# zhangxinsong-nlp/XFM

Measured on AMD Instinct MI355X. Metric: image-text pairs/sec fwd+bwd, XFM-base 224px/30tok, higher is better.
Workload: dtype bf16; 1 GPU; Pretrain.py full multimodal step (ITC+ITM+MLM+MIM), XFM-base, synthetic 224px images + 30-token captions, random init; units_per_gpu=64, global_batch=64, dropout=True, ordered_reductions=True, grad_allreduce=False, parallelism=dp1, image_res=224

## Files before the change

### xfm_amd/csrc/gemm_tn_256.hip

```cpp
__device__ __forceinline__ void wait_younger(int y) {
  if (y >= 3) asm volatile("s_waitcnt vmcnt(6)" ::: "memory");
  else if (y == 2) asm volatile("s_waitcnt vmcnt(4)" ::: "memory");
  else if (y == 1) asm volatile("s_waitcnt vmcnt(2)" ::: "memory");
  else asm volatile("s_waitcnt vmcnt(0)" ::: "memory");
}

struct Tn256Seg {
  const bf16* dY; const bf16* X;
  unsigned ldy, ldx;
  int n0, k0, mbeg, nk;
  bool do_bias;
  int rows;
};
__device__ __attribute__((aligned(16))) const unsigned tn_zero16[4] = {0u, 0u, 0u, 0u};

template <bool RAGGED>
__device__ __forceinline__ void tn256_mainloop(const Tn256Seg& sg, char* smem, f32x4 (&acc)[8][4], f32x4 (&bacc)[2]) {
  constexpr int UNIT = 64 * 256, BUF = 4 * UNIT;
  const int tid = threadIdx.x, lane = tid & 63, w = tid >> 6;
  const int wr = w >> 2, wc = w & 3;
  const int lr = lane & 15, lg = lane >> 4;
  const int n0 = sg.n0, k0 = sg.k0, mbeg = sg.mbeg, nk = sg.nk;
  const int total = 4 * nk;
  const bool do_bias = sg.do_bias;

  unsigned soff[4][2];
  int doff[4][2];
#pragma unroll
  for (int i = 0; i < 2; ++i) {
    const int b = i * 8 + w;
    const int r = 4 * b + (lane >> 4);
    const int c = ((lane & 15) ^ swz_t(r)) * 8;
    const unsigned rowy = (unsigned)(mbeg + r) * (unsigned)sg.ldy, rowx = (unsigned)(mbeg + r) * (unsigned)sg.ldx;
    soff[0][i] = rowy + n0 + (c >> 6) * 128 + (c & 63);
    soff[3][i] = rowy + n0 + (c >> 6) * 128 + 64 + (c & 63);
    soff[1][i] = rowx + k0 + (c >> 5) * 64 + (c & 31);
    soff[2][i] = rowx + k0 + (c >> 5) * 64 + 32 + (c & 31);
    doff[0][i] = 0 * UNIT + b * 1024;
    doff[1][i] = 1 * UNIT + b * 1024;
    doff[2][i] = 2 * UNIT + b * 1024;
    doff[3][i] = 3 * UNIT + b * 1024;
  }
  auto issue = [&](int s) {
    if (s >= total) return;
    const int kt = s >> 2, j = s & 3;
    char* base = smem + (kt & 1) * BUF;
    const bool isy = (j == 0 || j == 3);
    const bf16* src = (isy ? sg.dY : sg.X) + (size_t)kt * 64 * (size_t)(isy ? sg.ldy : sg.ldx);
#pragma unroll
    for (int i = 0; i < 2; ++i) {
      const unsigned so = j == 0 ? soff[0][i] : j == 1 ? soff[1][i] : j == 2 ? soff[2][i] : soff[3][i];
      const int dofs = j == 0 ? doff[0][i] : j == 1 ? doff[1][i] : j == 2 ? doff[2][i] : doff[3][i];
      const unsigned lds_addr = (unsigned)(uintptr_t)LDS_PTR(void, base) + (unsigned)__builtin_amdgcn_readfirstlane(dofs);
      const bf16* ptr = src + (size_t)so;
      if (RAGGED && kt * 64 + 4 * (i * 8 + w) + (lane >> 4) >= sg.rows) ptr = reinterpret_cast<const bf16*>(tn_zero16);
      asm volatile("s_mov_b32 m0, %1\n\ts_nop 0\n\tglobal_load_lds_dwordx4 %0, off" ::"v"(ptr), "s"(lds_addr) : "memory", "m0");
    }
  };

#pragma unroll
  for (int i = 0; i < 8; ++i)
#pragma unroll
    for (int j = 0; j < 4; ++j) acc[i][j] = f32x4{0.f, 0.f, 0.f, 0.f};
  bacc[0] = bacc[1] = f32x4{0.f, 0.f, 0.f, 0.f};
  bf16x8 ones;
#pragma unroll
  for (int i = 0; i < 8; ++i) ones[i] = f2bf(1.0f);

  const int lrow = 8 * lg + (lr >> 2);
  const int tsw = swz_t(lrow);
  int offa[4], offb[2];
#pragma unroll
  for (int f = 0; f < 4; ++f) {
    const int col = wr * 64 + f * 16 + 4 * (lr & 3);
    offa[f] = lrow * 256 + (((col >> 3) ^ tsw) << 4) + (col & 7) * 2;
  }
#pragma unroll
  for (int f = 0; f < 2; ++f) {
    const int col = wc * 32 + f * 16 + 4 * (lr & 3);
    offb[f] = lrow * 256 + (((col >> 3) ^ tsw) << 4) + (col & 7) * 2;
  }
  auto tr_pair = [&](const char* p) {
    const s16x4 lo = __builtin_amdgcn_ds_read_tr16_b64_v4i16(LDS_PTR(s16x4, p));
    const s16x4 hi = __builtin_amdgcn_ds_read_tr16_b64_v4i16(LDS_PTR(s16x4, p + 1024));
    union { struct { s16x4 a, b; } s; bf16x8 v; } u;
    u.s.a = lo;
    u.s.b = hi;
    return u.v;
  };
  bf16x8 xa[4][2], wb0[2][2], wb1[2][2];
  auto read_a = [&](const char* unit) {
#pragma unroll
    for (int f = 0; f < 4; ++f) {
      xa[f][0] = tr_pair(unit + offa[f]);
      xa[f][1] = tr_pair(unit + offa[f] + 8192);
    }
  };
  auto read_b = [&](const char* unit, bf16x8 (&wb)[2][2]) {
#pragma unroll
    for (int f = 0; f < 2; ++f) {
      wb[f][0] = tr_pair(unit + offb[f]);
      wb[f][1] = tr_pair(unit + offb[f] + 8192);
    }
  };
#define XFM_TQUAD(MH, NH, WB)                                                                                    \
  do {                                                                                                           \
    __builtin_amdgcn_s_setprio(1);                                                                               \
    _Pragma("unroll") for (int ks = 0; ks < 2; ++ks)                                                             \
    _Pragma("unroll") for (int m = 0; m < 4; ++m)                                                                \
    _Pragma("unroll") for (int n = 0; n < 2; ++n)                                                                \
      acc[MH * 4 + m][NH * 2 + n] =                                                                              \
          __builtin_amdgcn_mfma_f32_16x16x32_bf16(xa[m][ks], WB[n][ks], acc[MH * 4 + m][NH * 2 + n], 0, 0, 0);  \
    __builtin_amdgcn_s_setprio(0);                                                                               \
  } while (0)
#define XFM_TBIAS(H)                                                                                             \
  do {                                                                                                           \
    if (do_bias) {                                                                                               \
      _Pragma("unroll") for (int f = 0; f < 4; ++f)                                                              \
        if (f == wc) {                                                                                           \
          bacc[H] = __builtin_amdgcn_mfma_f32_16x16x32_bf16(xa[f][0], ones, bacc[H], 0, 0, 0);                  \
          bacc[H] = __builtin_amdgcn_mfma_f32_16x16x32_bf16(xa[f][1], ones, bacc[H], 0, 0, 0);                  \
        }                                                                                                        \
    }                                                                                                            \
  } while (0)

#pragma unroll
  for (int s = 0; s < 5; ++s) issue(s);
  wait_younger((total - 1 < 4 ? total - 1 : 4) - 1);
  XFM_BAR();
  if (wr == 1) XFM_BAR();

  for (int kt = 0; kt < nk; ++kt) {
    const char* buf = smem + (kt & 1) * BUF;
    const int ph = 4 * kt;
    int last;
    issue(ph + 5);
    read_a(buf + 0 * UNIT);
    read_b(buf + 1 * UNIT, wb0);
    last = ph + 5 < total ? ph + 5 : total - 1;
    wait_younger(last - (ph + 2));
    XFM_BAR();
    XFM_TQUAD(0, 0, wb0);
    XFM_TBIAS(0);
    XFM_BAR();
    issue(ph + 6);
    read_b(buf + 2 * UNIT, wb1);
    last = ph + 6 < total ? ph + 6 : total - 1;
    wait_younger(last - (ph + 3));
    XFM_BAR();
    XFM_TQUAD(0, 1, wb1);
    XFM_BAR();
    issue(ph + 7);
    read_a(buf + 3 * UNIT);
    XFM_BAR();
    XFM_TQUAD(1, 1, wb1);
    XFM_TBIAS(1);
    XFM_BAR();
    issue(ph + 8);
    last = ph + 8 < total ? ph + 8 : total - 1;
    wait_younger(last - (ph + 5) < 0 ? 0 : last - (ph + 5));
    XFM_BAR();
    XFM_TQUAD(1, 0, wb0);
    XFM_BAR();
  }
  if (wr == 0) XFM_BAR();
#undef XFM_TQUAD
#undef XFM_TBIAS

}

template <bool ATOMIC>
__device__ __forceinline__ void tn256_bias_out(float* dbias, int n0, const f32x4 (&bacc)[2]) {
  const int lane = threadIdx.x & 63, w = threadIdx.x >> 6, wr = w >> 2, wc = w & 3, lr = lane & 15, lg = lane >> 4;
  if (lr != 0) return;
#pragma unroll
  for (int h = 0; h < 2; ++h)
#pragma unroll
    for (int i = 0; i < 4; ++i) {
      float* d = dbias + n0 + wr * 128 + h * 64 + wc * 16 + 4 * lg + i;
      if (ATOMIC) atomicAdd(d, bacc[h][i]);
      else *d += bacc[h][i];
    }
}
__device__ __forceinline__ void tn256_bias_part(float* part, const f32x4 (&bacc)[2]) {
  const int lane = threadIdx.x & 63, w = threadIdx.x >> 6, wr = w >> 2, wc = w & 3, lr = lane & 15, lg = lane >> 4;
  if (lr != 0) return;
#pragma unroll
  for (int h = 0; h < 2; ++h) *reinterpret_cast<f32x4*>(part + wr * 128 + h * 64 + wc * 16 + 4 * lg) = bacc[h];
}
__device__ __forceinline__ void tn256_store_partial(float* ws, long slot, const f32x4 (&acc)[8][4]) {
  const int lane = threadIdx.x & 63, w = threadIdx.x >> 6;
  f32x4* wsp = reinterpret_cast<f32x4*>(ws) + ((slot * 8 + w) * 32) * 64 + lane;
#pragma unroll
  for (int nt = 0; nt < 8; ++nt)
#pragma unroll
    for (int kt = 0; kt < 4; ++kt) wsp[(nt * 4 + kt) * 64] = acc[nt][kt];
}
template <bool ATOMIC>
__device__ __forceinline__ void tn256_add_out(float* dW, long ldw, int n0, int k0, const f32x4 (&acc)[8][4]) {
  const int lane = threadIdx.x & 63, w = threadIdx.x >> 6, wr = w >> 2, wc = w & 3, lr = lane & 15, lg = lane >> 4;
#pragma unroll
  for (int nt = 0; nt < 8; ++nt)
#pragma unroll
    for (int kt = 0; kt < 4; ++kt) {
      const int k = k0 + wc * 64 + kt * 16 + lr;
#pragma unroll
      for (int rgi = 0; rgi < 4; ++rgi) {
        const int n = n0 + wr * 128 + nt * 16 + 4 * lg + rgi;
        if (ATOMIC) atomicAdd(dW + (long)n * ldw + k, acc[nt][kt][rgi]);
        else dW[(long)n * ldw + k] += acc[nt][kt][rgi];
      }
    }
}

__global__ __launch_bounds__(512) void gemm_tn_256_kernel(GemmTN g) {
  extern __shared__ __attribute__((aligned(16))) char smem[];
  const int tiles_k = g.K / 256, tiles_n = g.N / 256;
  const int per_split = tiles_k * tiles_n;
  const int wg = xcd_remap(blockIdx.x, gridDim.x);
  const int split = wg / per_split, t = wg % per_split;
  const int n0 = (t / tiles_k) * 256, k0 = (t % tiles_k) * 256;
  const int mbeg = split * g.m_per_split;
  int mend = mbeg + g.m_per_split;
  mend = mend < g.M ? mend : g.M;
  const Tn256Seg sg{g.dY, g.X, (unsigned)g.ldy, (unsigned)g.ldx, n0, k0, mbeg, (mend - mbeg) / 64, g.dbias != nullptr && k0 == 0, 0};
  f32x4 acc[8][4], bacc[2];
  tn256_mainloop<false>(sg, smem, acc, bacc);
  if (sg.do_bias) tn256_bias_out<true>(g.dbias, n0, bacc);
  if (g.ws != nullptr) {
    tn256_store_partial(g.ws, (long)split * per_split + t, acc);
    return;
  }
  tn256_add_out<true>(g.dW, g.ldw, n0, k0, acc);
}

#define TN_GROUP_MAX 48
struct TnGroupProb {
  const bf16* dY; const bf16* X;
  float* dW; float* dbias;
  unsigned ldy, ldx;
  long ldw;
  int tiles_k;
  int tile_end;
};
struct TnGroup {
  int nprob, nk;
  int M;
  int total_tiles, full_tiles;
  int sk_wgs;
  long sk_iters;
  float* ws;
  float* ws_bias;
  TnGroupProb p[TN_GROUP_MAX];
};
__host__ __device__ __forceinline__ long tn_sk_bound(long R, int nk, int sk_wgs, int i) {
  long raw = (long)i * R / sk_wgs;
  const int rem = (int)(raw % nk);
  if (rem < 4) raw -= rem;
  else if (nk - rem < 4) raw += nk - rem;
  return raw;
}

__global__ __launch_bounds__(512) void gemm_tn_group_kernel(TnGroup G) {
  extern __shared__ __attribute__((aligned(16))) char smem[];
  const int wg = xcd_remap(blockIdx.x, gridDim.x), nwg = gridDim.x;
  int dp_t = wg;
  long sk_pos = 0, sk_end = 0;
  if (wg < G.sk_wgs) {
    sk_pos = tn_sk_bound(G.sk_iters, G.nk, G.sk_wgs, wg);
    sk_end = tn_sk_bound(G.sk_iters, G.nk, G.sk_wgs, wg + 1);
  }
  const long sk_a = sk_pos;
  bool first = true;
  for (;;) {
    int tile, it0, it1;
    long slot = -1;
    if (dp_t < G.full_tiles) {
      tile = dp_t;
      dp_t += nwg;
      it0 = 0;
      it1 = G.nk;
    } else if (sk_pos < sk_end) {
      const int rt = (int)(sk_pos / G.nk);
      const long t_end = (long)(rt + 1) * G.nk;
      it0 = (int)(sk_pos - (long)rt * G.nk);
      it1 = (int)((sk_end < t_end ? sk_end : t_end) - (long)rt * G.nk);
      tile = G.full_tiles + rt;
      if (it0 != 0 || it1 != G.nk) slot = 2l * wg + (sk_pos == sk_a ? 0 : 1);
      sk_pos = (long)rt * G.nk + it1;
    } else {
      break;
    }
    if (!first) __syncthreads();
    first = false;
    int pi = 0;
    while (pi + 1 < G.nprob && tile >= G.p[pi].tile_end) ++pi;
    const TnGroupProb& P = G.p[pi];
    const int tl = tile - (pi > 0 ? G.p[pi - 1].tile_end : 0);
    const int n0 = (tl / P.tiles_k) * 256, k0 = (tl % P.tiles_k) * 256;
    const Tn256Seg sg{P.dY, P.X, P.ldy, P.ldx, n0, k0, it0 * 64, it1 - it0, P.dbias != nullptr && k0 == 0, G.M - it0 * 64};
    f32x4 acc[8][4], bacc[2];
    tn256_mainloop<true>(sg, smem, acc, bacc);
    if (slot >= 0) {
      if (sg.do_bias) tn256_bias_part(G.ws_bias + slot * 256, bacc);
      tn256_store_partial(G.ws, slot, acc);
    } else {
      if (sg.do_bias) tn256_bias_out<false>(P.dbias, n0, bacc);
      tn256_add_out<false>(P.dW, P.ldw, n0, k0, acc);
    }
  }
}

__global__ __launch_bounds__(256) void tn_group_fixup_kernel(TnGroup G) {
  const int rt = blockIdx.y;
  const int idx = blockIdx.x * 256 + threadIdx.x;
  const long R = G.sk_iters;
  const long a = (long)rt * G.nk, b = a + G.nk;
  int i0 = (int)(a * G.sk_wgs / R);
  i0 = i0 < G.sk_wgs - 1 ? i0 : G.sk_wgs - 1;
  while (i0 > 0 && tn_sk_bound(R, G.nk, G.sk_wgs, i0) > a) --i0;
  while (i0 + 1 < G.sk_wgs && tn_sk_bound(R, G.nk, G.sk_wgs, i0 + 1) <= a) ++i0;
  int i1 = i0;
  while (i1 + 1 < G.sk_wgs && tn_sk_bound(R, G.nk, G.sk_wgs, i1 + 1) < b) ++i1;
  if (i0 == i1) return;
  const f32x4* ws = reinterpret_cast<const f32x4*>(G.ws);
  f32x4 sum = f32x4{0.f, 0.f, 0.f, 0.f};
  for (int i = i0; i <= i1; ++i) {
    const long slot = 2l * i + (tn_sk_bound(R, G.nk, G.sk_wgs, i) >= a ? 0 : 1);
    sum += ws[slot * (8 * 32 * 64) + idx];
  }
  const int tile = G.full_tiles + rt;
  int pi = 0;
  while (pi + 1 < G.nprob && tile >= G.p[pi].tile_end) ++pi;
  const TnGroupProb& P = G.p[pi];
  const int tl = tile - (pi > 0 ? G.p[pi - 1].tile_end : 0);
  const int n0 = (tl / P.tiles_k) * 256, k0 = (tl % P.tiles_k) * 256;
  const int lane = idx & 63, q = (idx >> 6) & 31, w = idx >> 11;
  const int wr = w >> 2, wc = w & 3, lr = lane & 15, lg = lane >> 4, nt = q >> 2, kt = q & 3;
  const int k = k0 + wc * 64 + kt * 16 + lr;
  const int n = n0 + wr * 128 + nt * 16 + 4 * lg;
#pragma unroll
  for (int i = 0; i < 4; ++i) P.dW[(long)(n + i) * P.ldw + k] += sum[i];
  if (blockIdx.x == 0 && P.dbias != nullptr && k0 == 0) {
    float b = 0.f;
    for (int i = i0; i <= i1; ++i) {
      const long slot = 2l * i + (tn_sk_bound(R, G.nk, G.sk_wgs, i) >= a ? 0 : 1);
      b += G.ws_bias[slot * 256 + threadIdx.x];
    }
    P.dbias[n0 + threadIdx.x] += b;
  }
}

__global__ __launch_bounds__(256) void tn_reduce_kernel(const float* __restrict__ ws, float* __restrict__ dW, long ldw, int tiles_k,
                                                        int per_split, int splits) {
  const long idx = (long)blockIdx.x * 256 + threadIdx.x;
  const int lane = (int)(idx & 63), q = (int)((idx >> 6) & 31), w = (int)((idx >> 11) & 7);
  const int t = (int)(idx >> 14);
  if (t >= per_split) return;
  const f32x4* p = reinterpret_cast<const f32x4*>(ws) + idx;
  const long stride = (long)per_split * 8 * 32 * 64;
  f32x4 sum = p[0];
  for (int sp = 1; sp < splits; ++sp) {
    const f32x4 v = p[sp * stride];
    sum += v;
  }
  const int n0 = (t / tiles_k) * 256, k0 = (t % tiles_k) * 256;
  const int wr = w >> 2, wc = w & 3, lr = lane & 15, lg = lane >> 4, nt = q >> 2, kt = q & 3;
  const int k = k0 + wc * 64 + kt * 16 + lr;
  const int n = n0 + wr * 128 + nt * 16 + 4 * lg;
#pragma unroll
  for (int i = 0; i < 4; ++i) dW[(long)(n + i) * ldw + k] += sum[i];
}
```

Measured before the change: 1750 pairs/s.

## Deepen TN256 GEMM prefetch and interleave LDS fragment reads with MFMAs

```diff
diff --git a/xfm_amd/csrc/gemm_tn_256.hip b/xfm_amd/csrc/gemm_tn_256.hip
--- a/xfm_amd/csrc/gemm_tn_256.hip
+++ b/xfm_amd/csrc/gemm_tn_256.hip
@@ -4,6 +4,8 @@
   else if (y == 1) asm volatile("s_waitcnt vmcnt(2)" ::: "memory");
   else asm volatile("s_waitcnt vmcnt(0)" ::: "memory");
 }
+
+constexpr int TN256_D = 6;
 
 struct Tn256Seg {
   const bf16* dY; const bf16* X;
@@ -16,43 +18,29 @@
 
 template <bool RAGGED>
 __device__ __forceinline__ void tn256_mainloop(const Tn256Seg& sg, char* smem, f32x4 (&acc)[8][4], f32x4 (&bacc)[2]) {
-  constexpr int UNIT = 64 * 256, BUF = 4 * UNIT;
-  const int tid = threadIdx.x, lane = tid & 63, w = tid >> 6;
+  constexpr int UNIT = 64 * 256, BUF = 4 * UNIT, D = TN256_D;
+  const int tid = threadIdx.x, lane = tid & 63, w = __builtin_amdgcn_readfirstlane(tid >> 6);
   const int wr = w >> 2, wc = w & 3;
   const int lr = lane & 15, lg = lane >> 4;
   const int n0 = sg.n0, k0 = sg.k0, mbeg = sg.mbeg, nk = sg.nk;
   const int total = 4 * nk;
   const bool do_bias = sg.do_bias;
 
-  unsigned soff[4][2];
-  int doff[4][2];
-#pragma unroll
-  for (int i = 0; i < 2; ++i) {
-    const int b = i * 8 + w;
-    const int r = 4 * b + (lane >> 4);
-    const int c = ((lane & 15) ^ swz_t(r)) * 8;
-    const unsigned rowy = (unsigned)(mbeg + r) * (unsigned)sg.ldy, rowx = (unsigned)(mbeg + r) * (unsigned)sg.ldx;
-    soff[0][i] = rowy + n0 + (c >> 6) * 128 + (c & 63);
-    soff[3][i] = rowy + n0 + (c >> 6) * 128 + 64 + (c & 63);
-    soff[1][i] = rowx + k0 + (c >> 5) * 64 + (c & 31);
-    soff[2][i] = rowx + k0 + (c >> 5) * 64 + 32 + (c & 31);
-    doff[0][i] = 0 * UNIT + b * 1024;
-    doff[1][i] = 1 * UNIT + b * 1024;
-    doff[2][i] = 2 * UNIT + b * 1024;
-    doff[3][i] = 3 * UNIT + b * 1024;
-  }
+  const unsigned lds0 = (unsigned)(uintptr_t)LDS_PTR(void, smem);
+  const int r0 = 4 * w + (lane >> 4);
+  const int c0 = ((lane & 15) ^ swz_t(r0)) * 8;
+  const unsigned soy = (unsigned)(mbeg + r0) * sg.ldy + n0 + (c0 >> 6) * 128 + (c0 & 63);
+  const unsigned sox = (unsigned)(mbeg + r0) * sg.ldx + k0 + (c0 >> 5) * 64 + (c0 & 31);
   auto issue = [&](int s) {
     if (s >= total) return;
     const int kt = s >> 2, j = s & 3;
-    char* base = smem + (kt & 1) * BUF;
     const bool isy = (j == 0 || j == 3);
-    const bf16* src = (isy ? sg.dY : sg.X) + (size_t)kt * 64 * (size_t)(isy ? sg.ldy : sg.ldx);
+    const size_t ld = isy ? sg.ldy : sg.ldx;
+    const bf16* src = (isy ? sg.dY : sg.X) + (size_t)kt * 64 * ld + (j == 3 ? 64 : j == 2 ? 32 : 0);
 #pragma unroll
     for (int i = 0; i < 2; ++i) {
-      const unsigned so = j == 0 ? soff[0][i] : j == 1 ? soff[1][i] : j == 2 ? soff[2][i] : soff[3][i];
-      const int dofs = j == 0 ? doff[0][i] : j == 1 ? doff[1][i] : j == 2 ? doff[2][i] : doff[3][i];
-      const unsigned lds_addr = (unsigned)(uintptr_t)LDS_PTR(void, base) + (unsigned)__builtin_amdgcn_readfirstlane(dofs);
-      const bf16* ptr = src + (size_t)so;
+      const unsigned lds_addr = lds0 + (unsigned)((kt & 1) * BUF + j * UNIT + (i * 8 + w) * 1024);
+      const bf16* ptr = src + (size_t)i * 32 * ld + (size_t)(isy ? soy : sox);
       if (RAGGED && kt * 64 + 4 * (i * 8 + w) + (lane >> 4) >= sg.rows) ptr = reinterpret_cast<const bf16*>(tn_zero16);
       asm volatile("s_mov_b32 m0, %1\n\ts_nop 0\n\tglobal_load_lds_dwordx4 %0, off" ::"v"(ptr), "s"(lds_addr) : "memory", "m0");
     }
@@ -69,48 +57,39 @@
 
   const int lrow = 8 * lg + (lr >> 2);
   const int tsw = swz_t(lrow);
-  int offa[4], offb[2];
+  unsigned offa[4], offb[2];
 #pragma unroll
   for (int f = 0; f < 4; ++f) {
     const int col = wr * 64 + f * 16 + 4 * (lr & 3);
-    offa[f] = lrow * 256 + (((col >> 3) ^ tsw) << 4) + (col & 7) * 2;
+    offa[f] = lds0 + lrow * 256 + (((col >> 3) ^ tsw) << 4) + (col & 7) * 2;
   }
 #pragma unroll
   for (int f = 0; f < 2; ++f) {
     const int col = wc * 32 + f * 16 + 4 * (lr & 3);
-    offb[f] = lrow * 256 + (((col >> 3) ^ tsw) << 4) + (col & 7) * 2;
-  }
-  auto tr_pair = [&](const char* p) {
-    const s16x4 lo = __builtin_amdgcn_ds_read_tr16_b64_v4i16(LDS_PTR(s16x4, p));
-    const s16x4 hi = __builtin_amdgcn_ds_read_tr16_b64_v4i16(LDS_PTR(s16x4, p + 1024));
+    offb[f] = lds0 + lrow * 256 + (((col >> 3) ^ tsw) << 4) + (col & 7) * 2;
+  }
+  auto tr_pair = [&](unsigned a) {
+    const s16x4 lo = __builtin_amdgcn_ds_read_tr16_b64_v4i16(LDS_PTR(s16x4, (uintptr_t)a));
+    const s16x4 hi = __builtin_amdgcn_ds_read_tr16_b64_v4i16(LDS_PTR(s16x4, (uintptr_t)(a + 1024)));
     union { struct { s16x4 a, b; } s; bf16x8 v; } u;
     u.s.a = lo;
     u.s.b = hi;
     return u.v;
   };
   bf16x8 xa[4][2], wb0[2][2], wb1[2][2];
-  auto read_a = [&](const char* unit) {
-#pragma unroll
-    for (int f = 0; f < 4; ++f) {
-      xa[f][0] = tr_pair(unit + offa[f]);
-      xa[f][1] = tr_pair(unit + offa[f] + 8192);
-    }
-  };
-  auto read_b = [&](const char* unit, bf16x8 (&wb)[2][2]) {
-#pragma unroll
-    for (int f = 0; f < 2; ++f) {
-      wb[f][0] = tr_pair(unit + offb[f]);
-      wb[f][1] = tr_pair(unit + offb[f] + 8192);
-    }
-  };
-#define XFM_TQUAD(MH, NH, WB)                                                                                    \
+  auto frag_a = [&](int unit, int f, int ks) { return tr_pair(offa[f] + unit * UNIT + ks * 8192); };
+  auto frag_b = [&](int unit, int f, int ks) { return tr_pair(offb[f] + unit * UNIT + ks * 8192); };
+#define XFM_TQUAD(MH, NH, WB, BETWEEN)                                                                           \
   do {                                                                                                           \
     __builtin_amdgcn_s_setprio(1);                                                                               \
     _Pragma("unroll") for (int ks = 0; ks < 2; ++ks)                                                             \
     _Pragma("unroll") for (int m = 0; m < 4; ++m)                                                                \
-    _Pragma("unroll") for (int n = 0; n < 2; ++n)                                                                \
+    _Pragma("unroll") for (int n = 0; n < 2; ++n) {                                                              \
       acc[MH * 4 + m][NH * 2 + n] =                                                                              \
           __builtin_amdgcn_mfma_f32_16x16x32_bf16(xa[m][ks], WB[n][ks], acc[MH * 4 + m][NH * 2 + n], 0, 0, 0);  \
+      BETWEEN(ks * 8 + m * 2 + n);                                                                               \
+      __builtin_amdgcn_sched_barrier(0);                                                                         \
+    }                                                                                                            \
     __builtin_amdgcn_s_setprio(0);                                                                               \
   } while (0)
 #define XFM_TBIAS(H)                                                                                             \
@@ -123,46 +102,78 @@
         }                                                                                                        \
     }                                                                                                            \
   } while (0)
-
-#pragma unroll
-  for (int s = 0; s < 5; ++s) issue(s);
-  wait_younger((total - 1 < 4 ? total - 1 : 4) - 1);
+  auto wait_phase = [&](int q) {
+    const int last = q + D < total ? q + D : total - 1;
+    wait_younger(last - (q + 3) < 0 ? 0 : last - (q + 3));
+  };
+  auto hop = [](unsigned& off, int by) {
+    off += by;
+    asm volatile("" : "+v"(off));
+  };
+  auto ktile = [&](int kt, bf16x8 (&wbx)[2][2], bf16x8 (&wby)[2][2], int HOP) __attribute__((always_inline)) {
+    const int ph = 4 * kt;
+    issue(ph + D);
+#pragma unroll
+    for (int f = 0; f < 4; ++f) xa[f][1] = frag_a(0, f, 1);
+    wait_phase(ph);
+    XFM_BAR();
+    auto p0 = [&](int i) {
+      if (i < 8 && (i & 1) == 0) wby[(i >> 1) & 1][i >> 2] = frag_b(2, (i >> 1) & 1, i >> 2);
+    };
+    XFM_TQUAD(0, 0, wbx, p0);
+    XFM_TBIAS(0);
+    XFM_BAR();
+    issue(ph + 1 + D);
+    hop(offb[0], HOP);
+    hop(offb[1], HOP);
+    wait_phase(ph + 1);
+    XFM_BAR();
+    auto p1 = [&](int i) {
+      if (i >= 8 && (i & 1) == 0) xa[(i - 8) >> 1][0] = frag_a(3, (i - 8) >> 1, 0);
+    };
+    XFM_TQUAD(0, 1, wby, p1);
+    XFM_BAR();
+    issue(ph + 2 + D);
+#pragma unroll
+    for (int f = 0; f < 4; ++f) xa[f][1] = frag_a(3, f, 1);
+    wait_phase(ph + 2);
+    XFM_BAR();
+    auto p2 = [&](int) {};
+    XFM_TQUAD(1, 1, wby, p2);
+    XFM_TBIAS(1);
+    XFM_BAR();
+    issue(ph + 3 + D);
+#pragma unroll
+    for (int f = 0; f < 4; ++f) hop(offa[f], HOP);
+    wait_phase(ph + 3);
+    XFM_BAR();
+    auto p3 = [&](int i) {
+      if ((i & 1) != 0) return;
+      if (i < 8) wby[(i >> 1) & 1][i >> 2] = frag_b(1, (i >> 1) & 1, i >> 2);
+      else xa[(i - 8) >> 1][0] = frag_a(0, (i - 8) >> 1, 0);
+    };
+    XFM_TQUAD(1, 0, wbx, p3);
+    XFM_BAR();
+  };
+
+#pragma unroll
+  for (int s = 0; s < D; ++s) issue(s);
+  wait_phase(-1);
   XFM_BAR();
   if (wr == 1) XFM_BAR();
-
-  for (int kt = 0; kt < nk; ++kt) {
-    const char* buf = smem + (kt & 1) * BUF;
-    const int ph = 4 * kt;
-    int last;
-    issue(ph + 5);
-    read_a(buf + 0 * UNIT);
-    read_b(buf + 1 * UNIT, wb0);
-    last = ph + 5 < total ? ph + 5 : total - 1;
-    wait_younger(last - (ph + 2));
-    XFM_BAR();
-    XFM_TQUAD(0, 0, wb0);
-    XFM_TBIAS(0);
-    XFM_BAR();
-    issue(ph + 6);
-    read_b(buf + 2 * UNIT, wb1);
-    last = ph + 6 < total ? ph + 6 : total - 1;
-    wait_younger(last - (ph + 3));
-    XFM_BAR();
-    XFM_TQUAD(0, 1, wb1);
-    XFM_BAR();
-    issue(ph + 7);
-    read_a(buf + 3 * UNIT);
-    XFM_BAR();
-    XFM_TQUAD(1, 1, wb1);
-    XFM_TBIAS(1);
-    XFM_BAR();
-    issue(ph + 8);
-    last = ph + 8 < total ? ph + 8 : total - 1;
-    wait_younger(last - (ph + 5) < 0 ? 0 : last - (ph + 5));
-    XFM_BAR();
-    XFM_TQUAD(1, 0, wb0);
-    XFM_BAR();
-  }
+#pragma unroll
+  for (int f = 0; f < 4; ++f) xa[f][0] = frag_a(0, f, 0);
+#pragma unroll
+  for (int f = 0; f < 2; ++f) {
+    wb0[f][0] = frag_b(1, f, 0);
+    wb0[f][1] = frag_b(1, f, 1);
+  }
+  __builtin_amdgcn_s_waitcnt(0xc07f);
+  for (int kt = 0; kt + 1 < nk; kt += 2) {
+    ktile(kt, wb0, wb1, BUF);
+    ktile(kt + 1, wb1, wb0, -BUF);
+  }
+  if (nk & 1) ktile(nk - 1, wb0, wb1, BUF);
   if (wr == 0) XFM_BAR();
 #undef XFM_TQUAD
 #undef XFM_TBIAS
@@ -261,14 +272,18 @@
   return raw;
 }
 
+__device__ __forceinline__ long uniform_long(long v) {
+  return ((long)__builtin_amdgcn_readfirstlane((int)(v >> 32)) << 32) | (unsigned)__builtin_amdgcn_readfirstlane((int)v);
+}
+
 __global__ __launch_bounds__(512) void gemm_tn_group_kernel(TnGroup G) {
   extern __shared__ __attribute__((aligned(16))) char smem[];
   const int wg = xcd_remap(blockIdx.x, gridDim.x), nwg = gridDim.x;
   int dp_t = wg;
   long sk_pos = 0, sk_end = 0;
   if (wg < G.sk_wgs) {
-    sk_pos = tn_sk_bound(G.sk_iters, G.nk, G.sk_wgs, wg);
-    sk_end = tn_sk_bound(G.sk_iters, G.nk, G.sk_wgs, wg + 1);
+    sk_pos = uniform_long(tn_sk_bound(G.sk_iters, G.nk, G.sk_wgs, wg));
+    sk_end = uniform_long(tn_sk_bound(G.sk_iters, G.nk, G.sk_wgs, wg + 1));
   }
   const long sk_a = sk_pos;
   bool first = true;
```

After: 1761 pairs/s (median of 6 runs). Within noise of the previous version (+0.6%).
